# aliftffd/ViT-vs-Raw-IQ

Measured on AMD Instinct MI355X. Metric: IQ frames/sec training (fwd+loss+bwd+clip+AdamW), higher is better.
Workload: dtype bf16; 1 GPU; ViT-Tiny/16 224x224 C=1 19cls (BASELINE configs[1]); config_id=B, per_gpu_batch=256, global_batch=256, parallelism=dp1, hipgraph=True

## Files before the change

vit-vs-raw-iq_amd/csrc/attention.hip:

```cpp
#include <stdlib.h>

#include "common.h"
#include "iqvit.h"
#include "prof.h"

namespace {

constexpr int ATT_THREADS = 512;
constexpr int ATT_WAVES = ATT_THREADS / 64;
constexpr float LOG2E = 1.4426950408889634f;
constexpr float LN2 = 0.6931471805599453f;
constexpr float NEG_BIG = -1.0e30f;

__device__ __forceinline__ float fast_exp2(float x) { return __builtin_amdgcn_exp2f(x); }

template <int DH> struct AttCfg {
  static constexpr int LD = (DH == 16) ? 16 : DH + 16;
  static constexpr int KS = (DH + 31) / 32;
  static constexpr int DT = DH / 16;
  static constexpr int CPR = DH / 8;
};

typedef __attribute__((address_space(3))) s16x4 lds_s16x4;

__device__ __forceinline__ bf16x8 tr_frag(const bf16* tile, int ld, int r0, int c0, int lane) {
  const int i16 = lane & 15, g = lane >> 4;
  const bf16* a = tile + (r0 + 4 * g + (i16 >> 2)) * ld + c0 + 4 * (i16 & 3);
  s16x4 lo = __builtin_amdgcn_ds_read_tr16_b64_v4i16((lds_s16x4*)(a));
  s16x4 hi = __builtin_amdgcn_ds_read_tr16_b64_v4i16((lds_s16x4*)(a + 16 * ld));
  s16x8 v = {lo[0], lo[1], lo[2], lo[3], hi[0], hi[1], hi[2], hi[3]};
  return __builtin_bit_cast(bf16x8, v);
}

template <int DH>
__device__ __forceinline__ bf16x8 row_frag_lds(const bf16* tile, int row, int s, int lane) {
  const int d0 = s * 32 + 8 * (lane >> 4);
  bf16x8 v = {};
  if (DH >= 32 || d0 < DH) v = *reinterpret_cast<const bf16x8*>(tile + row * AttCfg<DH>::LD + d0);
  return v;
}
template <int DH>
__device__ __forceinline__ bf16x8 row_frag_gmem(const bf16* base, long ldg, int row, int nrows, int s, int lane) {
  const int d0 = s * 32 + 8 * (lane >> 4);
  bf16x8 v = {};
  if (row < nrows && (DH >= 32 || d0 < DH)) v = *reinterpret_cast<const bf16x8*>(base + (long)row * ldg + d0);
  return v;
}

template <int DH>
__device__ __forceinline__ void stage_rows(bf16* img, const bf16* base, long ldg, int r_begin, int nrows_pad, int S,
                                           int tid) {
  constexpr int CPR = AttCfg<DH>::CPR, LD = AttCfg<DH>::LD;
  for (int id = tid; id < nrows_pad * CPR; id += ATT_THREADS) {
    const int r = id / CPR, c = id % CPR;
    bf16x8 v = {};
    if (r_begin + r < S) v = *reinterpret_cast<const bf16x8*>(base + (long)(r_begin + r) * ldg + c * 8);
    *reinterpret_cast<bf16x8*>(img + r * LD + c * 8) = v;
  }
}

template <int DH, int UN>
__device__ __forceinline__ void stage_pair(bf16* imgA, const bf16* baseA, long ldgA, bf16* imgB, const bf16* baseB, long ldgB,
                                           int r_begin, int nrows_pad, int S, int tid) {
  constexpr int CPR = AttCfg<DH>::CPR, LD = AttCfg<DH>::LD;
  const int total = nrows_pad * CPR;
  for (int base = 0; base < total; base += UN * ATT_THREADS) {
    bf16x8 va[UN], vb[UN];
#pragma unroll
    for (int j = 0; j < UN; ++j) {
      const int id = min(base + j * ATT_THREADS + tid, total - 1);
      const int r = min(r_begin + id / CPR, S - 1), c = id % CPR;
      va[j] = *reinterpret_cast<const bf16x8*>(baseA + (long)r * ldgA + c * 8);
      vb[j] = *reinterpret_cast<const bf16x8*>(baseB + (long)r * ldgB + c * 8);
    }
#pragma unroll
    for (int j = 0; j < UN; ++j) {
      const int id = base + j * ATT_THREADS + tid;
      const int r = id / CPR, c = id % CPR;
      if (id < total) {
        const bool live = r_begin + r < S;
        *reinterpret_cast<bf16x8*>(imgA + r * LD + c * 8) = live ? va[j] : bf16x8{};
        *reinterpret_cast<bf16x8*>(imgB + r * LD + c * 8) = live ? vb[j] : bf16x8{};
      }
    }
  }
}

__device__ __forceinline__ bf16x8 pack_b(const f32x4& lo, const f32x4& hi) {
  bf16x8 v;
#pragma unroll
  for (int r = 0; r < 4; ++r) { v[r] = (bf16)lo[r]; v[4 + r] = (bf16)hi[r]; }
  return v;
}

__device__ __forceinline__ float group4_max(float v) {
  v = fmaxf(v, __shfl_xor(v, 16, 64));
  return fmaxf(v, __shfl_xor(v, 32, 64));
}
__device__ __forceinline__ float group4_sum(float v) {
  v += __shfl_xor(v, 16, 64);
  return v + __shfl_xor(v, 32, 64);
}

template <int DH, bool MASKED>
__global__ __launch_bounds__(ATT_THREADS) void attn_fwd_kernel(const bf16* __restrict__ qkv, bf16* __restrict__ out,
                                                               float* __restrict__ lse, const uint8_t* __restrict__ mask,
                                                               long mask_hstride, int S, int H, int kchunk,
                                                               float scale_log2, float masked_raw) {
  using C = AttCfg<DH>;
  extern __shared__ __attribute__((aligned(16))) unsigned char smem[];
  bf16* Ks = reinterpret_cast<bf16*>(smem);
  bf16* Vs = Ks + kchunk * C::LD;
  const int tid = threadIdx.x, lane = tid & 63, wave = tid >> 6, g = lane >> 4, c16 = lane & 15;
  const int b = blockIdx.x / H, h = blockIdx.x % H;
  const int D = H * DH;
  const long ldg = 3L * D;
  const bf16* qb = qkv + (long)b * S * ldg + h * DH;
  const bf16* kb_ = qb + D;
  const bf16* vb_ = qb + 2 * D;
  const uint8_t* mk = MASKED ? mask + (long)b * (mask_hstride ? (long)H * S * S : (long)S * S) + h * mask_hstride : nullptr;
  const int qtiles = (S + 31) / 32, npass = (qtiles + ATT_WAVES - 1) / ATT_WAVES, nstage = (S + kchunk - 1) / kchunk;

  if (nstage == 1) {
    stage_pair<DH, 4>(Ks, kb_, ldg, Vs, vb_, ldg, 0, min(kchunk, ((S + 31) / 32) * 32), S, tid);
    __syncthreads();
  }
  for (int pass = 0; pass < npass; ++pass) {
    const int qt = pass * ATT_WAVES + wave;
    const bool active = qt < qtiles;
    bf16x8 qf[2][C::KS];
    f32x4 o[2][C::DT];
    float m[2], lsum[2];
#pragma unroll
    for (int u = 0; u < 2; ++u) {
      m[u] = NEG_BIG; lsum[u] = 0.f;
#pragma unroll
      for (int s = 0; s < C::KS; ++s) qf[u][s] = row_frag_gmem<DH>(qb, ldg, qt * 32 + u * 16 + c16, active ? S : 0, s, lane);
#pragma unroll
      for (int dt = 0; dt < C::DT; ++dt) o[u][dt] = f32x4{0.f, 0.f, 0.f, 0.f};
    }
    for (int st = 0; st < nstage; ++st) {
      const int k0 = st * kchunk;
      const int krows = min(kchunk, ((S - k0 + 31) / 32) * 32);
      if (nstage > 1) {
        __syncthreads();
        stage_pair<DH, 2>(Ks, kb_, ldg, Vs, vb_, ldg, k0, krows, S, tid);
        __syncthreads();
      }
      if (active) {
        const bool u1 = qt * 32 + 16 < S;
        for (int kb = 0; kb < krows; kb += 32) {
          const bool k1 = k0 + kb + 16 < S;
          const bool kpad = k0 + kb + 32 > S;
          f32x4 sc[2][2];
#pragma unroll
          for (int kt = 0; kt < 2; ++kt) {
            if (kt == 1 && !k1) {
              sc[0][1] = f32x4{0.f, 0.f, 0.f, 0.f}; sc[1][1] = f32x4{0.f, 0.f, 0.f, 0.f};
              continue;
            }
            bf16x8 kf[C::KS];
#pragma unroll
            for (int s = 0; s < C::KS; ++s) kf[s] = row_frag_lds<DH>(Ks, kb + kt * 16 + c16, s, lane);
#pragma unroll
            for (int u = 0; u < 2; ++u) {
              f32x4 a = {0.f, 0.f, 0.f, 0.f};
              if (u == 0 || u1) {
#pragma unroll
                for (int s = 0; s < C::KS; ++s) a = __builtin_amdgcn_mfma_f32_16x16x32_bf16(kf[s], qf[u][s], a, 0, 0, 0);
              }
              sc[u][kt] = a;
            }
          }
          bf16x8 pb[2];
#pragma unroll
          for (int u = 0; u < 2; ++u) {
            if (u == 1 && !u1) { pb[1] = bf16x8{}; continue; }
            float mx = NEG_BIG;
#pragma unroll
            for (int kt = 0; kt < 2; ++kt) {
              if (kt == 1 && !k1) continue;
#pragma unroll
              for (int r = 0; r < 4; ++r) {
                float x = sc[u][kt][r];
                if (MASKED) {
                  const int key = k0 + kb + kt * 16 + 4 * g + r;
                  const int q = qt * 32 + u * 16 + c16;
                  if (key < S && q < S && !mk[(long)q * S + key]) x = masked_raw;
                }
                if (kpad) {
                  const int key = k0 + kb + kt * 16 + 4 * g + r;
                  x = key < S ? x : NEG_BIG;
                }
                sc[u][kt][r] = x;
                mx = fmaxf(mx, x);
              }
            }
            mx = group4_max(mx) * scale_log2;
            const float mn = fmaxf(m[u], mx);
            const float alpha = fast_exp2(m[u] - mn);
            m[u] = mn;
            float rs = 0.f;
#pragma unroll
            for (int kt = 0; kt < 2; ++kt) {
              if (kt == 1 && !k1) continue;
#pragma unroll
              for (int r = 0; r < 4; ++r) {
                const float pv = fast_exp2(fmaf(sc[u][kt][r], scale_log2, -mn));
                sc[u][kt][r] = pv;
                rs += pv;
              }
            }
            lsum[u] = lsum[u] * alpha + rs;
#pragma unroll
            for (int dt = 0; dt < C::DT; ++dt) o[u][dt] *= alpha;
            pb[u] = pack_b(sc[u][0], sc[u][1]);
          }
#pragma unroll
          for (int dt = 0; dt < C::DT; ++dt) {
            const bf16x8 vt = tr_frag(Vs, C::LD, kb, dt * 16, lane);
            o[0][dt] = __builtin_amdgcn_mfma_f32_16x16x32_bf16(vt, pb[0], o[0][dt], 0, 0, 0);
            if (u1) o[1][dt] = __builtin_amdgcn_mfma_f32_16x16x32_bf16(vt, pb[1], o[1][dt], 0, 0, 0);
          }
        }
      }
    }
    if (active) {
#pragma unroll
      for (int u = 0; u < 2; ++u) {
        const float l = group4_sum(lsum[u]);
        const float inv = 1.0f / l;
        const int q = qt * 32 + u * 16 + c16;
        if (q < S) {
#pragma unroll
          for (int dt = 0; dt < C::DT; ++dt) {
            bf16x4 w;
#pragma unroll
            for (int r = 0; r < 4; ++r) w[r] = (bf16)(o[u][dt][r] * inv);
            *reinterpret_cast<bf16x4*>(out + ((long)b * S + q) * D + h * DH + dt * 16 + 4 * g) = w;
          }
          if (g == 0) lse[((long)b * H + h) * S + q] = (m[u] + log2f(l)) * LN2;
        }
      }
    }
  }
}

template <int DH, bool MASKED>
__global__ __launch_bounds__(ATT_THREADS, 4) void attn_bwd_kernel(const bf16* __restrict__ qkv, const bf16* __restrict__ out,
                                                               const bf16* __restrict__ dout, const float* __restrict__ lse,
                                                               bf16* __restrict__ dqkv, const uint8_t* __restrict__ mask,
                                                               long mask_hstride, int S, int H, int spad, int chunk,
                                                               float scale, float masked_raw) {
  using C = AttCfg<DH>;
  extern __shared__ __attribute__((aligned(16))) unsigned char smem[];
  bf16* I0 = reinterpret_cast<bf16*>(smem);
  bf16* I1 = I0 + chunk * C::LD;
  float* lse_s = reinterpret_cast<float*>(I1 + chunk * C::LD);
  float* del_s = lse_s + spad;
  const int tid = threadIdx.x, lane = tid & 63, wave = tid >> 6, g = lane >> 4, c16 = lane & 15;
  const int b = blockIdx.x / H, h = blockIdx.x % H;
  const int D = H * DH;
  const long ldg = 3L * D;
  const bf16* qb = qkv + (long)b * S * ldg + h * DH;
  const bf16* kb_ = qb + D;
  const bf16* vb_ = qb + 2 * D;
  const bf16* ob = out + (long)b * S * D + h * DH;
  const bf16* dob = dout + (long)b * S * D + h * DH;
  bf16* dqb = dqkv + (long)b * S * ldg + h * DH;
  const uint8_t* mk = MASKED ? mask + (long)b * (mask_hstride ? (long)H * S * S : (long)S * S) + h * mask_hstride : nullptr;
  const float scale_log2 = scale * LOG2E;
  const int nblk = spad / 32;
  const int nchunk = (spad + chunk - 1) / chunk;
  const bool single = nchunk == 1;

  if (single) {
    stage_pair<DH, 4>(I0, qb, ldg, I1, dob, (long)D, 0, spad, S, tid);
    __syncthreads();
  }
  for (int q = tid; q < spad; q += ATT_THREADS) {
    float dl = 0.f, ls = 0.f;
    if (q < S) {
#pragma unroll
      for (int c = 0; c < C::CPR; ++c) {
        const bf16x8 a = single ? *reinterpret_cast<const bf16x8*>(I1 + q * C::LD + c * 8)
                                : *reinterpret_cast<const bf16x8*>(dob + (long)q * D + c * 8);
        const bf16x8 o8 = *reinterpret_cast<const bf16x8*>(ob + (long)q * D + c * 8);
#pragma unroll
        for (int e = 0; e < 8; ++e) dl += (float)a[e] * (float)o8[e];
      }
      ls = lse[((long)b * H + h) * S + q] * LOG2E;
    }
    del_s[q] = dl;
    lse_s[q] = ls;
  }
  __syncthreads();

  const int nunit = (S + 15) / 16;
  for (int ug = 0; ug * ATT_WAVES < nunit; ++ug) {
    const int unit = ug * ATT_WAVES + wave;
    const bool have = unit < nunit;
    bf16x8 kf[C::KS], vf[C::KS];
#pragma unroll
    for (int s = 0; s < C::KS; ++s) {
      kf[s] = row_frag_gmem<DH>(kb_, ldg, unit * 16 + c16, have ? S : 0, s, lane);
      vf[s] = row_frag_gmem<DH>(vb_, ldg, unit * 16 + c16, have ? S : 0, s, lane);
    }
    f32x4 dv[C::DT], dk[C::DT];
#pragma unroll
    for (int dt = 0; dt < C::DT; ++dt) { dv[dt] = f32x4{0.f, 0.f, 0.f, 0.f}; dk[dt] = f32x4{0.f, 0.f, 0.f, 0.f}; }
    const int key = unit * 16 + c16;
    const bool unit_partial = unit * 16 + 16 > S;
    for (int qc = 0; qc < nchunk; ++qc) {
      const int q0 = qc * chunk;
      const int rows = min(chunk, spad - q0);
      if (!single) {
        __syncthreads();
        stage_pair<DH, 2>(I0, qb, ldg, I1, dob, (long)D, q0, rows, S, tid);
        __syncthreads();
      }
      if (!have) continue;
      for (int ql = 0; ql < rows; ql += 32) {
        const bool u1 = q0 + ql + 16 < S;
        f32x4 p[2], ds[2];
#pragma unroll
        for (int u = 0; u < 2; ++u) {
          if (u == 1 && !u1) { p[1] = f32x4{0.f, 0.f, 0.f, 0.f}; ds[1] = f32x4{0.f, 0.f, 0.f, 0.f}; continue; }
          f32x4 sa = {0.f, 0.f, 0.f, 0.f}, dp = {0.f, 0.f, 0.f, 0.f};
#pragma unroll
          for (int s = 0; s < C::KS; ++s) {
            const bf16x8 qa = row_frag_lds<DH>(I0, ql + u * 16 + c16, s, lane);
            const bf16x8 da = row_frag_lds<DH>(I1, ql + u * 16 + c16, s, lane);
            sa = __builtin_amdgcn_mfma_f32_16x16x32_bf16(qa, kf[s], sa, 0, 0, 0);
            dp = __builtin_amdgcn_mfma_f32_16x16x32_bf16(da, vf[s], dp, 0, 0, 0);
          }
#pragma unroll
          for (int r = 0; r < 4; ++r) {
            const int q = q0 + ql + u * 16 + 4 * g + r;
            bool blocked = false;
            if (MASKED) blocked = q < S && key < S && !mk[(long)q * S + key];
            float pv = fast_exp2((blocked ? masked_raw : sa[r]) * scale_log2 - lse_s[q]);
            if (unit_partial) pv = key < S ? pv : 0.f;
            p[u][r] = pv;
            ds[u][r] = blocked ? 0.f : pv * (dp[r] - del_s[q]) * scale;
          }
        }
        const bf16x8 pB = pack_b(p[0], p[1]), dsB = pack_b(ds[0], ds[1]);
#pragma unroll
        for (int dt = 0; dt < C::DT; ++dt) {
          const bf16x8 doT = tr_frag(I1, C::LD, ql, dt * 16, lane);
          const bf16x8 qT = tr_frag(I0, C::LD, ql, dt * 16, lane);
          dv[dt] = __builtin_amdgcn_mfma_f32_16x16x32_bf16(doT, pB, dv[dt], 0, 0, 0);
          dk[dt] = __builtin_amdgcn_mfma_f32_16x16x32_bf16(qT, dsB, dk[dt], 0, 0, 0);
        }
      }
    }
    if (have && key < S) {
#pragma unroll
      for (int dt = 0; dt < C::DT; ++dt) {
        bf16x4 wk, wv;
#pragma unroll
        for (int r = 0; r < 4; ++r) { wk[r] = (bf16)dk[dt][r]; wv[r] = (bf16)dv[dt][r]; }
        *reinterpret_cast<bf16x4*>(dqb + (long)key * ldg + D + dt * 16 + 4 * g) = wk;
        *reinterpret_cast<bf16x4*>(dqb + (long)key * ldg + 2 * D + dt * 16 + 4 * g) = wv;
      }
    }
  }

  bf16x8 qf[2][C::KS], dof[2][C::KS];
  if (single) {
#pragma unroll
    for (int u = 0; u < 2; ++u)
#pragma unroll
      for (int s = 0; s < C::KS; ++s) {
        const int q = min(wave, nblk - 1) * 32 + u * 16 + c16;
        qf[u][s] = row_frag_lds<DH>(I0, q, s, lane);
        dof[u][s] = row_frag_lds<DH>(I1, q, s, lane);
      }
  }
  for (int qg = 0; qg * ATT_WAVES < nblk; ++qg) {
    const int qblk = qg * ATT_WAVES + wave;
    const bool have = qblk < nblk;
    float lq[2], dl[2];
#pragma unroll
    for (int u = 0; u < 2; ++u) {
      const int q = min(qblk, nblk - 1) * 32 + u * 16 + c16;
      if (!single || qg != 0) {
#pragma unroll
        for (int s = 0; s < C::KS; ++s) {
          qf[u][s] = row_frag_gmem<DH>(qb, ldg, q, have ? S : 0, s, lane);
          dof[u][s] = row_frag_gmem<DH>(dob, (long)D, q, have ? S : 0, s, lane);
        }
      }
      lq[u] = lse_s[q];
      dl[u] = del_s[q];
    }
    f32x4 dq[C::DT][2];
#pragma unroll
    for (int dt = 0; dt < C::DT; ++dt)
#pragma unroll
      for (int u = 0; u < 2; ++u) dq[dt][u] = f32x4{0.f, 0.f, 0.f, 0.f};
    for (int kc = 0; kc < nchunk; ++kc) {
      const int k0 = kc * chunk;
      const int rows = min(chunk, spad - k0);
      if (!single || qg == 0) {
        __syncthreads();
        stage_pair<DH, 2>(I0, kb_, ldg, I1, vb_, ldg, k0, rows, S, tid);
        __syncthreads();
      }
      if (!have) continue;
      const bool u1 = qblk * 32 + 16 < S;
      for (int kl = 0; kl < rows; kl += 32) {
        const bool kblk_partial = k0 + kl + 32 > S;
        const bool k1 = k0 + kl + 16 < S;
        f32x4 ds[2][2];
#pragma unroll
        for (int kt = 0; kt < 2; ++kt) {
          if (kt == 1 && !k1) { ds[0][1] = f32x4{0.f, 0.f, 0.f, 0.f}; ds[1][1] = f32x4{0.f, 0.f, 0.f, 0.f}; continue; }
          bf16x8 ka[C::KS], va[C::KS];
#pragma unroll
          for (int s = 0; s < C::KS; ++s) {
            ka[s] = row_frag_lds<DH>(I0, kl + kt * 16 + c16, s, lane);
            va[s] = row_frag_lds<DH>(I1, kl + kt * 16 + c16, s, lane);
          }
#pragma unroll
          for (int u = 0; u < 2; ++u) {
            if (u == 1 && !u1) { ds[1][kt] = f32x4{0.f, 0.f, 0.f, 0.f}; continue; }
            f32x4 sa = {0.f, 0.f, 0.f, 0.f}, dp = {0.f, 0.f, 0.f, 0.f};
#pragma unroll
            for (int s = 0; s < C::KS; ++s) {
              sa = __builtin_amdgcn_mfma_f32_16x16x32_bf16(ka[s], qf[u][s], sa, 0, 0, 0);
              dp = __builtin_amdgcn_mfma_f32_16x16x32_bf16(va[s], dof[u][s], dp, 0, 0, 0);
            }
#pragma unroll
            for (int r = 0; r < 4; ++r) {
              const int key = k0 + kl + kt * 16 + 4 * g + r;
              bool blocked = false;
              if (MASKED) {
                const int q = qblk * 32 + u * 16 + c16;
                blocked = q < S && key < S && !mk[(long)q * S + key];
              }
              float pv = fast_exp2((blocked ? masked_raw : sa[r]) * scale_log2 - lq[u]);
              if (kblk_partial) pv = key < S ? pv : 0.f;
              ds[u][kt][r] = blocked ? 0.f : pv * (dp[r] - dl[u]) * scale;
            }
          }
        }
        bf16x8 dsB[2];
#pragma unroll
        for (int u = 0; u < 2; ++u) dsB[u] = pack_b(ds[u][0], ds[u][1]);
#pragma unroll
        for (int dt = 0; dt < C::DT; ++dt) {
          const bf16x8 kT = tr_frag(I0, C::LD, kl, dt * 16, lane);
          dq[dt][0] = __builtin_amdgcn_mfma_f32_16x16x32_bf16(kT, dsB[0], dq[dt][0], 0, 0, 0);
          if (u1) dq[dt][1] = __builtin_amdgcn_mfma_f32_16x16x32_bf16(kT, dsB[1], dq[dt][1], 0, 0, 0);
        }
      }
    }
    if (have) {
#pragma unroll
      for (int u = 0; u < 2; ++u) {
        const int q = qblk * 32 + u * 16 + c16;
        if (q < S) {
#pragma unroll
          for (int dt = 0; dt < C::DT; ++dt) {
            bf16x4 w;
#pragma unroll
            for (int r = 0; r < 4; ++r) w[r] = (bf16)dq[dt][u][r];
            *reinterpret_cast<bf16x4*>(dqb + (long)q * ldg + dt * 16 + 4 * g) = w;
          }
        }
      }
    }
  }
}

constexpr int ONCE_MAX_SPAD = 224;
constexpr int ONCE_LD = 64;

__device__ __forceinline__ int once_off(int row, int col) { return row * ONCE_LD + (col ^ (((row >> 1) & 3) << 4)); }

__device__ __forceinline__ bf16x8 once_tr_frag(const bf16* tile, int r0, int dt, int lane) {
  const int i16 = lane & 15, g = lane >> 4;
  const bf16* a = tile + once_off(r0 + 4 * g + (i16 >> 2), dt * 16 + 4 * (i16 & 3));
  s16x4 lo = __builtin_amdgcn_ds_read_tr16_b64_v4i16((lds_s16x4*)(a));
  s16x4 hi = __builtin_amdgcn_ds_read_tr16_b64_v4i16((lds_s16x4*)(a + 16 * ONCE_LD));
  s16x8 v = {lo[0], lo[1], lo[2], lo[3], hi[0], hi[1], hi[2], hi[3]};
  return __builtin_bit_cast(bf16x8, v);
}
__device__ __forceinline__ bf16x8 once_row_frag(const bf16* tile, int row, int s, int lane) {
  return *reinterpret_cast<const bf16x8*>(tile + once_off(row, s * 32 + 8 * (lane >> 4)));
}

template <int NT, int UN, int NIMG>
__device__ __forceinline__ void once_stage(bf16* const (&img)[NIMG], const bf16* const (&base)[NIMG],
                                           const long (&ldg)[NIMG], int spad, int S, int tid) {
  const int total = spad * 8;
  for (int b0 = 0; b0 < total; b0 += UN * NT) {
    bf16x8 v[NIMG][UN];
#pragma unroll
    for (int j = 0; j < UN; ++j) {
      const int id = min(b0 + j * NT + tid, total - 1);
      const int r = min(id >> 3, S - 1), c = id & 7;
#pragma unroll
      for (int i = 0; i < NIMG; ++i) v[i][j] = *reinterpret_cast<const bf16x8*>(base[i] + (long)r * ldg[i] + c * 8);
    }
#pragma unroll
    for (int j = 0; j < UN; ++j) {
      const int id = b0 + j * NT + tid;
      const int r = id >> 3, c = id & 7;
      if (id < total) {
        const bool live = r < S;
#pragma unroll
        for (int i = 0; i < NIMG; ++i) *reinterpret_cast<bf16x8*>(img[i] + once_off(r, c * 8)) = live ? v[i][j] : bf16x8{};
      }
    }
  }
}

template <int NT>
__global__ __launch_bounds__(NT, 4) void attn_bwd_once_kernel(const bf16* __restrict__ qkv, const bf16* __restrict__ out,
                                                              const bf16* __restrict__ dout, const float* __restrict__ lse,
                                                              bf16* __restrict__ dqkv, int S, int H, int spad, float scale) {
  constexpr int DH = 64, KS = 2, DT = 4, NW = NT / 64;
  extern __shared__ __attribute__((aligned(16))) unsigned char smem[];
  bf16* I0 = reinterpret_cast<bf16*>(smem);
  bf16* I1 = I0 + spad * ONCE_LD;
  float* lse_s = reinterpret_cast<float*>(I1 + spad * ONCE_LD);
  float* del_s = lse_s + spad;
  bf16* dSi = reinterpret_cast<bf16*>(del_s + spad);
  const int tid = threadIdx.x, lane = tid & 63, wave = tid >> 6, g = lane >> 4, c16 = lane & 15;
  const int b = blockIdx.x / H, h = blockIdx.x % H;
  const int D = H * DH;
  const long ldg = 3L * D;
  const bf16* qb = qkv + (long)b * S * ldg + h * DH;
  const bf16* kb_ = qb + D;
  const bf16* vb_ = qb + 2 * D;
  const bf16* ob = out + (long)b * S * D + h * DH;
  const bf16* dob = dout + (long)b * S * D + h * DH;
  bf16* dqb = dqkv + (long)b * S * ldg + h * DH;
  const float scale_log2 = scale * LOG2E;
  const int nunit = (S + 15) / 16;
  const int ldS = nunit * 16 + 8;

  {
    bf16* const img[2] = {I0, I1};
    const bf16* const src[2] = {qb, dob};
    const long lds_[2] = {ldg, (long)D};
    once_stage<NT, 2048 / NT, 2>(img, src, lds_, spad, S, tid);
  }
  __syncthreads();
  for (int q = tid; q < spad; q += NT) {
    float dl = 0.f, ls = 0.f;
    if (q < S) {
#pragma unroll
      for (int c = 0; c < 8; ++c) {
        const bf16x8 a = *reinterpret_cast<const bf16x8*>(I1 + once_off(q, c * 8));
        const bf16x8 o8 = *reinterpret_cast<const bf16x8*>(ob + (long)q * D + c * 8);
#pragma unroll
        for (int e = 0; e < 8; ++e) dl += (float)a[e] * (float)o8[e];
      }
      ls = lse[((long)b * H + h) * S + q] * LOG2E;
    }
    del_s[q] = dl;
    lse_s[q] = ls;
  }
  __syncthreads();

  for (int unit = wave; unit < nunit; unit += NW) {
    bf16x8 kf[KS], vf[KS];
#pragma unroll
    for (int s = 0; s < KS; ++s) {
      kf[s] = row_frag_gmem<DH>(kb_, ldg, unit * 16 + c16, S, s, lane);
      vf[s] = row_frag_gmem<DH>(vb_, ldg, unit * 16 + c16, S, s, lane);
    }
    f32x4 dv[DT], dk[DT];
#pragma unroll
    for (int dt = 0; dt < DT; ++dt) { dv[dt] = f32x4{0.f, 0.f, 0.f, 0.f}; dk[dt] = f32x4{0.f, 0.f, 0.f, 0.f}; }
    const int key = unit * 16 + c16;
    const bool unit_partial = unit * 16 + 16 > S;
    for (int ql = 0; ql < spad; ql += 32) {
      const bool u1 = ql + 16 < S;
      f32x4 p[2], ds[2];
#pragma unroll
      for (int u = 0; u < 2; ++u) {
        if (u == 1 && !u1) { p[1] = f32x4{0.f, 0.f, 0.f, 0.f}; ds[1] = f32x4{0.f, 0.f, 0.f, 0.f}; continue; }
        f32x4 sa = {0.f, 0.f, 0.f, 0.f}, dp = {0.f, 0.f, 0.f, 0.f};
#pragma unroll
        for (int s = 0; s < KS; ++s) {
          const bf16x8 qa = once_row_frag(I0, ql + u * 16 + c16, s, lane);
          const bf16x8 da = once_row_frag(I1, ql + u * 16 + c16, s, lane);
          sa = __builtin_amdgcn_mfma_f32_16x16x32_bf16(qa, kf[s], sa, 0, 0, 0);
          dp = __builtin_amdgcn_mfma_f32_16x16x32_bf16(da, vf[s], dp, 0, 0, 0);
        }
        const f32x4 lq4 = *reinterpret_cast<const f32x4*>(lse_s + ql + u * 16 + 4 * g);
        const f32x4 dl4 = *reinterpret_cast<const f32x4*>(del_s + ql + u * 16 + 4 * g);
#pragma unroll
        for (int r = 0; r < 4; ++r) {
          float pv = fast_exp2(sa[r] * scale_log2 - lq4[r]);
          if (unit_partial) pv = key < S ? pv : 0.f;
          p[u][r] = pv;
          ds[u][r] = pv * (dp[r] - dl4[r]) * scale;
        }
      }
      const bf16x8 pB = pack_b(p[0], p[1]), dsB = pack_b(ds[0], ds[1]);
      bf16* w = dSi + (ql + 4 * g) * ldS + key;
#pragma unroll
      for (int r = 0; r < 4; ++r) w[r * ldS] = dsB[r];
      if (u1) {
#pragma unroll
        for (int r = 0; r < 4; ++r) w[(16 + r) * ldS] = dsB[4 + r];
      }
#pragma unroll
      for (int dt = 0; dt < DT; ++dt) {
        const bf16x8 doT = once_tr_frag(I1, ql, dt, lane);
        const bf16x8 qT = once_tr_frag(I0, ql, dt, lane);
        dv[dt] = __builtin_amdgcn_mfma_f32_16x16x32_bf16(doT, pB, dv[dt], 0, 0, 0);
        dk[dt] = __builtin_amdgcn_mfma_f32_16x16x32_bf16(qT, dsB, dk[dt], 0, 0, 0);
      }
    }
    if (key < S) {
#pragma unroll
      for (int dt = 0; dt < DT; ++dt) {
        bf16x4 wk, wv;
#pragma unroll
        for (int r = 0; r < 4; ++r) { wk[r] = (bf16)dk[dt][r]; wv[r] = (bf16)dv[dt][r]; }
        *reinterpret_cast<bf16x4*>(dqb + (long)key * ldg + D + dt * 16 + 4 * g) = wk;
        *reinterpret_cast<bf16x4*>(dqb + (long)key * ldg + 2 * D + dt * 16 + 4 * g) = wv;
      }
    }
  }

  __syncthreads();
  {
    bf16* const img[1] = {I0};
    const bf16* const src[1] = {kb_};
    const long lds_[1] = {ldg};
    once_stage<NT, 2048 / NT, 1>(img, src, lds_, spad, S, tid);
  }
  __syncthreads();
  for (int half = wave; half < nunit; half += NW) {
    const int q = half * 16 + c16;
    const bf16* drow = dSi + q * ldS + 4 * g;
    f32x4 dq[DT];
#pragma unroll
    for (int dt = 0; dt < DT; ++dt) dq[dt] = f32x4{0.f, 0.f, 0.f, 0.f};
    for (int kl = 0; kl < spad; kl += 32) {
      const bool k1 = kl + 16 < S;
      const bf16x4 lo = *reinterpret_cast<const bf16x4*>(drow + kl);
      bf16x4 hi = {};
      if (k1) hi = *reinterpret_cast<const bf16x4*>(drow + kl + 16);
      const bf16x8 dsB = {lo[0], lo[1], lo[2], lo[3], hi[0], hi[1], hi[2], hi[3]};
#pragma unroll
      for (int dt = 0; dt < DT; ++dt) {
        const bf16x8 kT = once_tr_frag(I0, kl, dt, lane);
        dq[dt] = __builtin_amdgcn_mfma_f32_16x16x32_bf16(kT, dsB, dq[dt], 0, 0, 0);
      }
    }
    if (q < S) {
#pragma unroll
      for (int dt = 0; dt < DT; ++dt) {
        bf16x4 w;
#pragma unroll
        for (int r = 0; r < 4; ++r) w[r] = (bf16)dq[dt][r];
        *reinterpret_cast<bf16x4*>(dqb + (long)q * ldg + dt * 16 + 4 * g) = w;
      }
    }
  }
}

template <int DH>
__device__ __forceinline__ bf16x8 row_frag_img(const bf16* tile, int ld, int row, int s, int lane) {
  const int d0 = s * 32 + 8 * (lane >> 4);
  bf16x8 v = {};
  if (DH >= 32 || d0 < DH) v = *reinterpret_cast<const bf16x8*>(tile + row * ld + d0);
  return v;
}

template <int UN>
__device__ __forceinline__ void stage_block(bf16* img, int ld, const bf16* src, int cols, int S, int spad, int tid, int nthr) {
  const int cpr = cols >> 3, total = spad * cpr, live = S * cpr;
  for (int base = 0; base < total; base += UN * nthr) {
    bf16x8 v[UN];
#pragma unroll
    for (int j = 0; j < UN; ++j) {
      const int id = min(base + j * nthr + tid, live - 1);
      v[j] = *reinterpret_cast<const bf16x8*>(src + (long)id * 8);
    }
#pragma unroll
    for (int j = 0; j < UN; ++j) {
      const int id = base + j * nthr + tid;
      if (id < total) {
        const int r = id / cpr, c = id - r * cpr;
        *reinterpret_cast<bf16x8*>(img + r * ld + c * 8) = id < live ? v[j] : bf16x8{};
      }
    }
  }
}

template <int DH, int G>
__global__ __launch_bounds__(ATT_THREADS) void attn_frame_fwd_kernel(const bf16* __restrict__ qkv, bf16* __restrict__ out,
                                                                     float* __restrict__ lse, int S, int H, int spad,
                                                                     float scale_log2) {
  using C = AttCfg<DH>;
  extern __shared__ __attribute__((aligned(16))) unsigned char smem[];
  bf16* img = reinterpret_cast<bf16*>(smem);
  const int tid = threadIdx.x, lane = tid & 63, wave = tid >> 6, g = lane >> 4, c16 = lane & 15;
  const int nwave = blockDim.x >> 6;
  const int b = blockIdx.x;
  const int D = H * DH, ld = 3 * D + 16;
  stage_block<8>(img, ld, qkv + (long)b * S * 3 * D, 3 * D, S, spad, tid, blockDim.x);
  __syncthreads();
  const int qtiles = (S + 31) / 32;
  for (int h = wave; h < H; h += nwave) {
    const bf16* Qs = img + h * DH;
    const bf16* Ks = Qs + D;
    const bf16* Vs = Qs + 2 * D;
    for (int qt0 = 0; qt0 < qtiles; qt0 += G) {
      bf16x8 qf[G][2][C::KS];
      f32x4 o[G][2][C::DT];
      float m[G][2], lsum[G][2];
      bool live[G][2];
#pragma unroll
      for (int t = 0; t < G; ++t)
#pragma unroll
        for (int u = 0; u < 2; ++u) {
          const int q0 = (qt0 + t) * 32 + u * 16;
          live[t][u] = q0 < S;
          m[t][u] = NEG_BIG; lsum[t][u] = 0.f;
#pragma unroll
          for (int s = 0; s < C::KS; ++s) qf[t][u][s] = row_frag_img<DH>(Qs, ld, min(q0 + c16, spad - 1), s, lane);
#pragma unroll
          for (int dt = 0; dt < C::DT; ++dt) o[t][u][dt] = f32x4{0.f, 0.f, 0.f, 0.f};
        }
      for (int kb = 0; kb < spad; kb += 32) {
        const bool k1 = kb + 16 < S;
        bf16x8 kf[2][C::KS], vt[C::DT];
#pragma unroll
        for (int kt = 0; kt < 2; ++kt)
#pragma unroll
          for (int s = 0; s < C::KS; ++s) kf[kt][s] = row_frag_img<DH>(Ks, ld, kb + kt * 16 + c16, s, lane);
#pragma unroll
        for (int dt = 0; dt < C::DT; ++dt) vt[dt] = tr_frag(Vs, ld, kb, dt * 16, lane);
#pragma unroll
        for (int t = 0; t < G; ++t)
#pragma unroll
          for (int u = 0; u < 2; ++u) {
            if (!live[t][u]) continue;
            f32x4 sc[2];
#pragma unroll
            for (int kt = 0; kt < 2; ++kt) {
              f32x4 a = {0.f, 0.f, 0.f, 0.f};
              if (kt == 0 || k1) {
#pragma unroll
                for (int s = 0; s < C::KS; ++s) a = __builtin_amdgcn_mfma_f32_16x16x32_bf16(kf[kt][s], qf[t][u][s], a, 0, 0, 0);
              }
              sc[kt] = a;
            }
            float mx = NEG_BIG;
#pragma unroll
            for (int kt = 0; kt < 2; ++kt) {
              if (kt == 1 && !k1) { sc[1] = f32x4{0.f, 0.f, 0.f, 0.f}; continue; }
#pragma unroll
              for (int r = 0; r < 4; ++r) {
                const int key = kb + kt * 16 + 4 * g + r;
                const float x = key < S ? sc[kt][r] : NEG_BIG;
                sc[kt][r] = x;
                mx = fmaxf(mx, x);
              }
            }
            mx = group4_max(mx) * scale_log2;
            const float mn = fmaxf(m[t][u], mx);
            const float alpha = fast_exp2(m[t][u] - mn);
            m[t][u] = mn;
            float rs = 0.f;
#pragma unroll
            for (int kt = 0; kt < 2; ++kt) {
              if (kt == 1 && !k1) continue;
#pragma unroll
              for (int r = 0; r < 4; ++r) {
                const float pv = fast_exp2(fmaf(sc[kt][r], scale_log2, -mn));
                sc[kt][r] = pv;
                rs += pv;
              }
            }
            lsum[t][u] = lsum[t][u] * alpha + rs;
            const bf16x8 pb = pack_b(sc[0], sc[1]);
#pragma unroll
            for (int dt = 0; dt < C::DT; ++dt) {
              o[t][u][dt] *= alpha;
              o[t][u][dt] = __builtin_amdgcn_mfma_f32_16x16x32_bf16(vt[dt], pb, o[t][u][dt], 0, 0, 0);
            }
          }
      }
#pragma unroll
      for (int t = 0; t < G; ++t)
#pragma unroll
        for (int u = 0; u < 2; ++u) {
          if (!live[t][u]) continue;
          const float l = group4_sum(lsum[t][u]);
          const float inv = 1.0f / l;
          const int q = (qt0 + t) * 32 + u * 16 + c16;
          if (q < S) {
#pragma unroll
            for (int dt = 0; dt < C::DT; ++dt) {
              bf16x4 w;
#pragma unroll
              for (int r = 0; r < 4; ++r) w[r] = (bf16)(o[t][u][dt][r] * inv);
              *reinterpret_cast<bf16x4*>(out + ((long)b * S + q) * D + h * DH + dt * 16 + 4 * g) = w;
            }
            if (g == 0) lse[((long)b * H + h) * S + q] = (m[t][u] + log2f(l)) * LN2;
          }
        }
    }
  }
}

template <int DH, int UG, int QG>
__global__ __launch_bounds__(ATT_THREADS) void attn_frame_bwd_kernel(const bf16* __restrict__ qkv, const bf16* __restrict__ out,
                                                                     const bf16* __restrict__ dout, const float* __restrict__ lse,
                                                                     bf16* __restrict__ dqkv, int S, int H, int spad, float scale) {
  using C = AttCfg<DH>;
  extern __shared__ __attribute__((aligned(16))) unsigned char smem[];
  const int tid = threadIdx.x, lane = tid & 63, wave = tid >> 6, g = lane >> 4, c16 = lane & 15;
  const int nwave = blockDim.x >> 6;
  const int b = blockIdx.x;
  const int D = H * DH, ld = 3 * D + 16, ldo = D + 16;
  bf16* img = reinterpret_cast<bf16*>(smem);
  bf16* dimg = img + spad * ld;
  float* lse_s = reinterpret_cast<float*>(dimg + spad * ldo);
  float* del_s = lse_s + H * spad;
  const long ldg = 3L * D;
  const float scale_log2 = scale * LOG2E;
  for (int id = tid; id < spad * H; id += blockDim.x) {
    const int q = id / H, h = id - q * H;
    float dl = 0.f, ls = 0.f;
    if (q < S) {
      const bf16* orow = out + ((long)b * S + q) * D + h * DH;
      const bf16* drow = dout + ((long)b * S + q) * D + h * DH;
#pragma unroll
      for (int c = 0; c < C::CPR; ++c) {
        const bf16x8 a = *reinterpret_cast<const bf16x8*>(drow + c * 8);
        const bf16x8 o8 = *reinterpret_cast<const bf16x8*>(orow + c * 8);
#pragma unroll
        for (int e = 0; e < 8; ++e) dl += (float)a[e] * (float)o8[e];
      }
      ls = lse[((long)b * H + h) * S + q] * LOG2E;
    }
    del_s[h * spad + q] = dl;
    lse_s[h * spad + q] = ls;
  }
  stage_block<8>(img, ld, qkv + (long)b * S * ldg, 3 * D, S, spad, tid, blockDim.x);
  stage_block<4>(dimg, ldo, dout + (long)b * S * D, D, S, spad, tid, blockDim.x);
  __syncthreads();
  bf16* dqb = dqkv + (long)b * S * ldg;
  const int nunit = (S + 15) / 16, nblk = spad / 32;
  for (int h = wave; h < H; h += nwave) {
    const bf16* Qs = img + h * DH;
    const bf16* Ks = Qs + D;
    const bf16* Vs = Qs + 2 * D;
    const bf16* Os = dimg + h * DH;
    const float* lq_s = lse_s + h * spad;
    const float* dl_s = del_s + h * spad;
    for (int un0 = 0; un0 < nunit; un0 += UG) {
      bf16x8 kf[UG][C::KS], vf[UG][C::KS];
      f32x4 dv[UG][C::DT], dk[UG][C::DT];
#pragma unroll
      for (int j = 0; j < UG; ++j) {
        const int row = min((un0 + j) * 16 + c16, spad - 1);
#pragma unroll
        for (int s = 0; s < C::KS; ++s) {
          kf[j][s] = row_frag_img<DH>(Ks, ld, row, s, lane);
          vf[j][s] = row_frag_img<DH>(Vs, ld, row, s, lane);
        }
#pragma unroll
        for (int dt = 0; dt < C::DT; ++dt) { dv[j][dt] = f32x4{0.f, 0.f, 0.f, 0.f}; dk[j][dt] = f32x4{0.f, 0.f, 0.f, 0.f}; }
      }
      for (int ql = 0; ql < spad; ql += 32) {
        const bool u1 = ql + 16 < S;
        bf16x8 qa[2][C::KS], da[2][C::KS], doT[C::DT], qT[C::DT];
        f32x4 lq4[2], dl4[2];
#pragma unroll
        for (int u = 0; u < 2; ++u) {
#pragma unroll
          for (int s = 0; s < C::KS; ++s) {
            qa[u][s] = row_frag_img<DH>(Qs, ld, ql + u * 16 + c16, s, lane);
            da[u][s] = row_frag_img<DH>(Os, ldo, ql + u * 16 + c16, s, lane);
          }
          lq4[u] = *reinterpret_cast<const f32x4*>(lq_s + ql + u * 16 + 4 * g);
          dl4[u] = *reinterpret_cast<const f32x4*>(dl_s + ql + u * 16 + 4 * g);
        }
#pragma unroll
        for (int dt = 0; dt < C::DT; ++dt) {
          doT[dt] = tr_frag(Os, ldo, ql, dt * 16, lane);
          qT[dt] = tr_frag(Qs, ld, ql, dt * 16, lane);
        }
#pragma unroll
        for (int j = 0; j < UG; ++j) {
          const int unit = un0 + j;
          if (unit >= nunit) continue;
          const int key = unit * 16 + c16;
          const bool unit_partial = unit * 16 + 16 > S;
          f32x4 p[2], ds[2];
#pragma unroll
          for (int u = 0; u < 2; ++u) {
            if (u == 1 && !u1) { p[1] = f32x4{0.f, 0.f, 0.f, 0.f}; ds[1] = f32x4{0.f, 0.f, 0.f, 0.f}; continue; }
            f32x4 sa = {0.f, 0.f, 0.f, 0.f}, dp = {0.f, 0.f, 0.f, 0.f};
#pragma unroll
            for (int s = 0; s < C::KS; ++s) {
              sa = __builtin_amdgcn_mfma_f32_16x16x32_bf16(qa[u][s], kf[j][s], sa, 0, 0, 0);
              dp = __builtin_amdgcn_mfma_f32_16x16x32_bf16(da[u][s], vf[j][s], dp, 0, 0, 0);
            }
#pragma unroll
            for (int r = 0; r < 4; ++r) {
              float pv = fast_exp2(sa[r] * scale_log2 - lq4[u][r]);
              if (unit_partial) pv = key < S ? pv : 0.f;
              p[u][r] = pv;
              ds[u][r] = pv * (dp[r] - dl4[u][r]) * scale;
            }
          }
          const bf16x8 pB = pack_b(p[0], p[1]), dsB = pack_b(ds[0], ds[1]);
#pragma unroll
          for (int dt = 0; dt < C::DT; ++dt) {
            dv[j][dt] = __builtin_amdgcn_mfma_f32_16x16x32_bf16(doT[dt], pB, dv[j][dt], 0, 0, 0);
            dk[j][dt] = __builtin_amdgcn_mfma_f32_16x16x32_bf16(qT[dt], dsB, dk[j][dt], 0, 0, 0);
          }
        }
      }
#pragma unroll
      for (int j = 0; j < UG; ++j) {
        const int key = (un0 + j) * 16 + c16;
        if (un0 + j < nunit && key < S) {
#pragma unroll
          for (int dt = 0; dt < C::DT; ++dt) {
            bf16x4 wk, wv;
#pragma unroll
            for (int r = 0; r < 4; ++r) { wk[r] = (bf16)dk[j][dt][r]; wv[r] = (bf16)dv[j][dt][r]; }
            *reinterpret_cast<bf16x4*>(dqb + (long)key * ldg + D + h * DH + dt * 16 + 4 * g) = wk;
            *reinterpret_cast<bf16x4*>(dqb + (long)key * ldg + 2 * D + h * DH + dt * 16 + 4 * g) = wv;
          }
        }
      }
    }
    for (int qb0 = 0; qb0 < nblk; qb0 += QG) {
      bf16x8 qf[QG][2][C::KS], dof[QG][2][C::KS];
      float lq[QG][2], dl[QG][2];
      bool live[QG][2];
      f32x4 dq[QG][C::DT][2];
#pragma unroll
      for (int t = 0; t < QG; ++t)
#pragma unroll
        for (int u = 0; u < 2; ++u) {
          const int q0 = (qb0 + t) * 32 + u * 16;
          live[t][u] = q0 < S;
          const int q = min(q0 + c16, spad - 1);
#pragma unroll
          for (int s = 0; s < C::KS; ++s) {
            qf[t][u][s] = row_frag_img<DH>(Qs, ld, q, s, lane);
            dof[t][u][s] = row_frag_img<DH>(Os, ldo, q, s, lane);
          }
          lq[t][u] = lq_s[q];
          dl[t][u] = dl_s[q];
#pragma unroll
          for (int dt = 0; dt < C::DT; ++dt) dq[t][dt][u] = f32x4{0.f, 0.f, 0.f, 0.f};
        }
      for (int kl = 0; kl < spad; kl += 32) {
        const bool kblk_partial = kl + 32 > S;
        const bool k1 = kl + 16 < S;
        bf16x8 ka[2][C::KS], va[2][C::KS], kT[C::DT];
#pragma unroll
        for (int kt = 0; kt < 2; ++kt)
#pragma unroll
          for (int s = 0; s < C::KS; ++s) {
            ka[kt][s] = row_frag_img<DH>(Ks, ld, kl + kt * 16 + c16, s, lane);
            va[kt][s] = row_frag_img<DH>(Vs, ld, kl + kt * 16 + c16, s, lane);
          }
#pragma unroll
        for (int dt = 0; dt < C::DT; ++dt) kT[dt] = tr_frag(Ks, ld, kl, dt * 16, lane);
#pragma unroll
        for (int t = 0; t < QG; ++t)
#pragma unroll
          for (int u = 0; u < 2; ++u) {
            if (!live[t][u]) continue;
            f32x4 ds[2];
#pragma unroll
            for (int kt = 0; kt < 2; ++kt) {
              if (kt == 1 && !k1) { ds[1] = f32x4{0.f, 0.f, 0.f, 0.f}; continue; }
              f32x4 sa = {0.f, 0.f, 0.f, 0.f}, dp = {0.f, 0.f, 0.f, 0.f};
#pragma unroll
              for (int s = 0; s < C::KS; ++s) {
                sa = __builtin_amdgcn_mfma_f32_16x16x32_bf16(ka[kt][s], qf[t][u][s], sa, 0, 0, 0);
                dp = __builtin_amdgcn_mfma_f32_16x16x32_bf16(va[kt][s], dof[t][u][s], dp, 0, 0, 0);
              }
#pragma unroll
              for (int r = 0; r < 4; ++r) {
                const int key = kl + kt * 16 + 4 * g + r;
                float pv = fast_exp2(sa[r] * scale_log2 - lq[t][u]);
                if (kblk_partial) pv = key < S ? pv : 0.f;
                ds[kt][r] = pv * (dp[r] - dl[t][u]) * scale;
              }
            }
            const bf16x8 dsB = pack_b(ds[0], ds[1]);
#pragma unroll
            for (int dt = 0; dt < C::DT; ++dt)
              dq[t][dt][u] = __builtin_amdgcn_mfma_f32_16x16x32_bf16(kT[dt], dsB, dq[t][dt][u], 0, 0, 0);
          }
      }
#pragma unroll
      for (int t = 0; t < QG; ++t)
#pragma unroll
        for (int u = 0; u < 2; ++u) {
          const int q = (qb0 + t) * 32 + u * 16 + c16;
          if (live[t][u] && q < S) {
#pragma unroll
            for (int dt = 0; dt < C::DT; ++dt) {
              bf16x4 w;
#pragma unroll
              for (int r = 0; r < 4; ++r) w[r] = (bf16)dq[t][dt][u][r];
              *reinterpret_cast<bf16x4*>(dqb + (long)q * ldg + h * DH + dt * 16 + 4 * g) = w;
            }
          }
        }
    }
  }
}

constexpr size_t ATT_FRAME_LDS_MAX = 112 * 1024;
inline size_t frame_fwd_lds(int S, int H, int dh) {
  const int spad = (S + 31) / 32 * 32;
  return (size_t)spad * (3 * H * dh + 16) * 2;
}
inline size_t frame_bwd_lds(int S, int H, int dh) {
  const int spad = (S + 31) / 32 * 32;
  return (size_t)spad * (3 * H * dh + 16) * 2 + (size_t)spad * (H * dh + 16) * 2 + (size_t)2 * H * spad * sizeof(float);
}
inline bool use_frame(int S, size_t lds) {
  static const int tune = [] { const char* e = getenv("IQ_TUNE_ATTN_FRAME"); return e ? atoi(e) : -1; }();
  if (lds > ATT_FRAME_LDS_MAX) return false;
  if (tune == 0) return false;
  if (tune == 1) return true;
  return S <= 128;
}

template <int DH>
int launch_frame_fwd(const void* qkv, void* out, float* lse, int B, int S, int H, hipStream_t st) {
  const int spad = (S + 31) / 32 * 32;
  const size_t lds = frame_fwd_lds(S, H, DH);
  auto k = attn_frame_fwd_kernel<DH, (DH == 64 ? 2 : 4)>;
  if (lds > 48 * 1024) (void)hipFuncSetAttribute((const void*)k, hipFuncAttributeMaxDynamicSharedMemorySize, (int)lds);
  const int threads = 64 * (H < ATT_WAVES ? H : ATT_WAVES);
  k<<<B, threads, lds, st>>>((const bf16*)qkv, (bf16*)out, lse, S, H, spad, LOG2E / sqrtf((float)DH));
  return iq_launch_status();
}
template <int DH>
int launch_frame_bwd(const void* qkv, const void* out, const void* dout, const float* lse, void* dqkv, int B, int S, int H,
                     hipStream_t st) {
  const int spad = (S + 31) / 32 * 32;
  const size_t lds = frame_bwd_lds(S, H, DH);
  auto k = attn_frame_bwd_kernel<DH, (DH == 64 ? 2 : 3), (DH == 16 ? 4 : DH == 32 ? 3 : 2)>;
  if (lds > 48 * 1024) (void)hipFuncSetAttribute((const void*)k, hipFuncAttributeMaxDynamicSharedMemorySize, (int)lds);
  const int threads = 64 * (H < ATT_WAVES ? H : ATT_WAVES);
  k<<<B, threads, lds, st>>>((const bf16*)qkv, (const bf16*)out, (const bf16*)dout, lse, (bf16*)dqkv, S, H, spad,
                             1.0f / sqrtf((float)DH));
  return iq_launch_status();
}

constexpr size_t ATT_LDS_FWD_BUDGET = 72 * 1024;
constexpr size_t ATT_LDS_BWD_BUDGET = 76 * 1024;
constexpr int ATT_MAX_S = 4096;

template <int DH> int bwd_chunk_rows(int S) {
  const int spad = (S + 31) / 32 * 32;
  const long room = (long)ATT_LDS_BWD_BUDGET - (long)2 * spad * sizeof(float);
  int chunk = (int)(room / (2 * AttCfg<DH>::LD * 2)) / 32 * 32;
  if (chunk > spad) chunk = spad;
  return chunk;
}
template <int DH> size_t bwd_lds_bytes(int S) {
  const int spad = (S + 31) / 32 * 32;
  return (size_t)2 * bwd_chunk_rows<DH>(S) * AttCfg<DH>::LD * 2 + (size_t)2 * spad * sizeof(float);
}

template <int DH, bool MASKED>
int launch_fwd(const void* qkv, void* out, float* lse, const uint8_t* mask, long mask_hstride, int B, int S, int H,
               hipStream_t st) {
  const int spad = (S + 31) / 32 * 32;
  int kchunk = (int)(ATT_LDS_FWD_BUDGET / (2 * AttCfg<DH>::LD * 2)) / 32 * 32;
  if (kchunk > spad) kchunk = spad;
  const size_t lds = (size_t)2 * kchunk * AttCfg<DH>::LD * 2;
  const float scale_log2 = LOG2E / sqrtf((float)DH);
  if (lds > 48 * 1024)
    (void)hipFuncSetAttribute((const void*)attn_fwd_kernel<DH, MASKED>, hipFuncAttributeMaxDynamicSharedMemorySize, (int)lds);
  attn_fwd_kernel<DH, MASKED><<<B * H, ATT_THREADS, lds, st>>>((const bf16*)qkv, (bf16*)out, lse, mask, mask_hstride, S, H,
                                                               kchunk, scale_log2, -10000.0f * sqrtf((float)DH));
  return iq_launch_status();
}

template <int DH, bool MASKED>
int launch_bwd(const void* qkv, const void* out, const void* dout, const float* lse, void* dqkv, const uint8_t* mask,
               long mask_hstride, int B, int S, int H, hipStream_t st) {
  const int spad = (S + 31) / 32 * 32;
  const int chunk = bwd_chunk_rows<DH>(S);
  if (S > ATT_MAX_S || chunk < 32) return IQ_ERR_UNSUPPORTED;
  const size_t lds = bwd_lds_bytes<DH>(S);
  if (lds > 48 * 1024)
    (void)hipFuncSetAttribute((const void*)attn_bwd_kernel<DH, MASKED>, hipFuncAttributeMaxDynamicSharedMemorySize, (int)lds);
  attn_bwd_kernel<DH, MASKED><<<B * H, ATT_THREADS, lds, st>>>((const bf16*)qkv, (const bf16*)out, (const bf16*)dout, lse,
                                                               (bf16*)dqkv, mask, mask_hstride, S, H, spad, chunk,
                                                               1.0f / sqrtf((float)DH), -10000.0f * sqrtf((float)DH));
  return iq_launch_status();
}

inline int once_threads(int S, int dh, bool masked) {
  static const int tune = [] { const char* e = getenv("IQ_TUNE_ATTN_BWD_ONCE"); return e ? atoi(e) : -1; }();
  if (masked || dh != 64 || (S + 31) / 32 * 32 > ONCE_MAX_SPAD || tune == 0) return 0;
  return tune == 512 ? 512 : 1024;
}
template <int NT>
int launch_bwd_once(const void* qkv, const void* out, const void* dout, const float* lse, void* dqkv, int B, int S, int H,
                    hipStream_t st) {
  const int spad = (S + 31) / 32 * 32, nunit = (S + 15) / 16;
  const size_t lds = (size_t)2 * spad * ONCE_LD * 2 + (size_t)2 * spad * sizeof(float) + (size_t)spad * (nunit * 16 + 8) * 2;
  auto k = attn_bwd_once_kernel<NT>;
  if (lds > 48 * 1024) (void)hipFuncSetAttribute((const void*)k, hipFuncAttributeMaxDynamicSharedMemorySize, (int)lds);
  k<<<B * H, NT, lds, st>>>((const bf16*)qkv, (const bf16*)out, (const bf16*)dout, lse, (bf16*)dqkv, S, H, spad,
                            1.0f / sqrtf(64.0f));
  return iq_launch_status();
}

template <bool MASKED>
int dispatch_fwd(const void* qkv, void* out, float* lse, const uint8_t* mask, long hs, int B, int S, int H, int dh,
                 hipStream_t st) {
  switch (dh) {
    case 16: return launch_fwd<16, MASKED>(qkv, out, lse, mask, hs, B, S, H, st);
    case 32: return launch_fwd<32, MASKED>(qkv, out, lse, mask, hs, B, S, H, st);
    case 64: return launch_fwd<64, MASKED>(qkv, out, lse, mask, hs, B, S, H, st);
    default: return IQ_ERR_UNSUPPORTED;
  }
}
template <bool MASKED>
int dispatch_bwd(const void* qkv, const void* out, const void* dout, const float* lse, void* dqkv, const uint8_t* mask,
                 long hs, int B, int S, int H, int dh, hipStream_t st) {
  switch (dh) {
    case 16: return launch_bwd<16, MASKED>(qkv, out, dout, lse, dqkv, mask, hs, B, S, H, st);
    case 32: return launch_bwd<32, MASKED>(qkv, out, dout, lse, dqkv, mask, hs, B, S, H, st);
    case 64: return launch_bwd<64, MASKED>(qkv, out, dout, lse, dqkv, mask, hs, B, S, H, st);
    default: return IQ_ERR_UNSUPPORTED;
  }
}

}

extern "C" int iq_attn_supported(int S, int dh) {
  if (S <= 0 || S > ATT_MAX_S) return 0;
  return (dh == 16 || dh == 32 || dh == 64) ? 1 : 0;
}

extern "C" int iq_attn_fwd_masked(const void* qkv, void* out, float* lse, const uint8_t* mask, long mask_hstride, int B,
                                  int S, int H, int dh, iq_stream_t stream) {
  if (B <= 0) return IQ_OK;
  if (!qkv || !out || !lse || S <= 0 || H <= 0) return IQ_ERR_ARG;
  if (mask_hstride != 0 && mask_hstride != (long)S * S) return IQ_ERR_ARG;
  hipStream_t st = (hipStream_t)stream;
  IQ_PROF(IQ_FAM_ATTN_FWD, st);
  const bool frame = !mask && (dh == 16 || dh == 32 || dh == 64) && use_frame(S, frame_fwd_lds(S, H, dh));
  {
    const double rows = (double)B * S, Dm = (double)H * dh;
    if (frame) IQ_PROF_K(2.0 * rows * 4.0 * Dm + 4.0 * B * H * S, 4.0 * B * H * (double)S * S * dh, "attn_frame_fwd_kernel<%d>", dh);
    else IQ_PROF_K(2.0 * rows * 4.0 * Dm + 4.0 * B * H * S, 4.0 * B * H * (double)S * S * dh, "attn_fwd_kernel<%d, %s>", dh, mask ? "true" : "false");
  }
  if (frame) {
    switch (dh) {
      case 16: return launch_frame_fwd<16>(qkv, out, lse, B, S, H, st);
      case 32: return launch_frame_fwd<32>(qkv, out, lse, B, S, H, st);
      default: return launch_frame_fwd<64>(qkv, out, lse, B, S, H, st);
    }
  }
  return mask ? dispatch_fwd<true>(qkv, out, lse, mask, mask_hstride, B, S, H, dh, st)
              : dispatch_fwd<false>(qkv, out, lse, nullptr, 0, B, S, H, dh, st);
}
extern "C" int iq_attn_fwd(const void* qkv, void* out, float* lse, int B, int S, int H, int dh, iq_stream_t stream) {
  return iq_attn_fwd_masked(qkv, out, lse, nullptr, 0, B, S, H, dh, stream);
}

extern "C" int iq_attn_bwd_masked(const void* qkv, const void* out, const void* dout, const float* lse, void* dqkv,
                                  const uint8_t* mask, long mask_hstride, int B, int S, int H, int dh,
                                  iq_stream_t stream) {
  if (B <= 0) return IQ_OK;
  if (!qkv || !out || !dout || !lse || !dqkv || S <= 0 || H <= 0) return IQ_ERR_ARG;
  if (mask_hstride != 0 && mask_hstride != (long)S * S) return IQ_ERR_ARG;
  hipStream_t st = (hipStream_t)stream;
  IQ_PROF(IQ_FAM_ATTN_BWD, st);
  const bool frame = !mask && (dh == 16 || dh == 32 || dh == 64) && use_frame(S, frame_bwd_lds(S, H, dh));
  const int once = frame ? 0 : once_threads(S, dh, mask != nullptr);
  {
    const double rows = (double)B * S, Dm = (double)H * dh;
    if (frame) IQ_PROF_K(2.0 * rows * 8.0 * Dm + 4.0 * B * H * S, 14.0 * B * H * (double)S * S * dh, "attn_frame_bwd_kernel<%d>", dh);
    else if (once) IQ_PROF_K(2.0 * rows * 8.0 * Dm + 4.0 * B * H * S, 10.0 * B * H * (double)S * S * dh, "attn_bwd_once_kernel<%d>", once);
    else IQ_PROF_K(2.0 * rows * 8.0 * Dm + 4.0 * B * H * S, 14.0 * B * H * (double)S * S * dh, "attn_bwd_kernel<%d, %s>", dh, mask ? "true" : "false");
  }
  if (frame) {
    switch (dh) {
      case 16: return launch_frame_bwd<16>(qkv, out, dout, lse, dqkv, B, S, H, st);
      case 32: return launch_frame_bwd<32>(qkv, out, dout, lse, dqkv, B, S, H, st);
      default: return launch_frame_bwd<64>(qkv, out, dout, lse, dqkv, B, S, H, st);
    }
  }
  if (once == 512) return launch_bwd_once<512>(qkv, out, dout, lse, dqkv, B, S, H, st);
  if (once) return launch_bwd_once<1024>(qkv, out, dout, lse, dqkv, B, S, H, st);
  return mask ? dispatch_bwd<true>(qkv, out, dout, lse, dqkv, mask, mask_hstride, B, S, H, dh, st)
              : dispatch_bwd<false>(qkv, out, dout, lse, dqkv, nullptr, 0, B, S, H, dh, st);
}
extern "C" int iq_attn_bwd(const void* qkv, const void* out, const void* dout, const float* lse, void* dqkv, int B,
                           int S, int H, int dh, iq_stream_t stream) {
  return iq_attn_bwd_masked(qkv, out, dout, lse, dqkv, nullptr, 0, B, S, H, dh, stream);
}
```

Baseline: 52430 frames/s.

## Prefetch K/V fragments, O tile and LSE early in attention backward kernel

```diff
diff --git a/vit-vs-raw-iq_amd/csrc/attention.hip b/vit-vs-raw-iq_amd/csrc/attention.hip
--- a/vit-vs-raw-iq_amd/csrc/attention.hip
+++ b/vit-vs-raw-iq_amd/csrc/attention.hip
@@ -495,26 +495,42 @@
 template <int NT, int UN, int NIMG>
 __device__ __forceinline__ void once_stage(bf16* const (&img)[NIMG], const bf16* const (&base)[NIMG],
                                            const long (&ldg)[NIMG], int spad, int S, int tid) {
+  static_assert(UN * NT >= ONCE_MAX_SPAD * 8, "one trip covers an image");
   const int total = spad * 8;
-  for (int b0 = 0; b0 < total; b0 += UN * NT) {
-    bf16x8 v[NIMG][UN];
-#pragma unroll
-    for (int j = 0; j < UN; ++j) {
-      const int id = min(b0 + j * NT + tid, total - 1);
-      const int r = min(id >> 3, S - 1), c = id & 7;
-#pragma unroll
-      for (int i = 0; i < NIMG; ++i) v[i][j] = *reinterpret_cast<const bf16x8*>(base[i] + (long)r * ldg[i] + c * 8);
-    }
-#pragma unroll
-    for (int j = 0; j < UN; ++j) {
-      const int id = b0 + j * NT + tid;
-      const int r = id >> 3, c = id & 7;
-      if (id < total) {
-        const bool live = r < S;
-#pragma unroll
-        for (int i = 0; i < NIMG; ++i) *reinterpret_cast<bf16x8*>(img[i] + once_off(r, c * 8)) = live ? v[i][j] : bf16x8{};
-      }
-    }
+  bf16x8 v[NIMG][UN];
+#pragma unroll
+  for (int j = 0; j < UN; ++j) {
+    const int id = min(j * NT + tid, total - 1);
+    const int r = min(id >> 3, S - 1), c = id & 7;
+#pragma unroll
+    for (int i = 0; i < NIMG; ++i) v[i][j] = *reinterpret_cast<const bf16x8*>(base[i] + (long)r * ldg[i] + c * 8);
+  }
+#pragma unroll
+  for (int j = 0; j < UN; ++j) {
+    const int id = j * NT + tid;
+    const int r = id >> 3, c = id & 7;
+    if (id < total) {
+      const bool live = r < S;
+#pragma unroll
+      for (int i = 0; i < NIMG; ++i) *reinterpret_cast<bf16x8*>(img[i] + once_off(r, c * 8)) = live ? v[i][j] : bf16x8{};
+    }
+  }
+}
+template <int NT, int UN>
+__device__ __forceinline__ void once_request(bf16x8 (&v)[UN], const bf16* base, long ldg, int spad, int S, int tid) {
+#pragma unroll
+  for (int j = 0; j < UN; ++j) {
+    const int id = min(j * NT + tid, spad * 8 - 1);
+    v[j] = *reinterpret_cast<const bf16x8*>(base + (long)min(id >> 3, S - 1) * ldg + (id & 7) * 8);
+  }
+}
+template <int NT, int UN>
+__device__ __forceinline__ void once_write(bf16* img, const bf16x8 (&v)[UN], int spad, int S, int tid) {
+#pragma unroll
+  for (int j = 0; j < UN; ++j) {
+    const int id = j * NT + tid;
+    const int r = id >> 3, c = id & 7;
+    if (id < spad * 8) *reinterpret_cast<bf16x8*>(img + once_off(r, c * 8)) = r < S ? v[j] : bf16x8{};
   }
 }
 
@@ -522,7 +538,7 @@
 __global__ __launch_bounds__(NT, 4) void attn_bwd_once_kernel(const bf16* __restrict__ qkv, const bf16* __restrict__ out,
                                                               const bf16* __restrict__ dout, const float* __restrict__ lse,
                                                               bf16* __restrict__ dqkv, int S, int H, int spad, float scale) {
-  constexpr int DH = 64, KS = 2, DT = 4, NW = NT / 64;
+  constexpr int DH = 64, KS = 2, DT = 4, NW = NT / 64, UN = 2048 / NT;
   extern __shared__ __attribute__((aligned(16))) unsigned char smem[];
   bf16* I0 = reinterpret_cast<bf16*>(smem);
   bf16* I1 = I0 + spad * ONCE_LD;
@@ -543,41 +559,57 @@
   const int nunit = (S + 15) / 16;
   const int ldS = nunit * 16 + 8;
 
+  bf16x8 kf[KS], vf[KS];
+  if (wave < nunit) {
+    const long row = min(wave * 16 + c16, S - 1);
+#pragma unroll
+    for (int s = 0; s < KS; ++s) {
+      kf[s] = *reinterpret_cast<const bf16x8*>(kb_ + row * ldg + s * 32 + 8 * g);
+      vf[s] = *reinterpret_cast<const bf16x8*>(vb_ + row * ldg + s * 32 + 8 * g);
+    }
+  }
+  const int per = (spad + NW - 1) / NW;
+  const int qd = lane < per ? wave * per + lane : spad;
+  const float ls_pre = lse[((long)b * H + h) * S + min(qd, S - 1)];
   {
-    bf16* const img[2] = {I0, I1};
-    const bf16* const src[2] = {qb, dob};
-    const long lds_[2] = {ldg, (long)D};
-    once_stage<NT, 2048 / NT, 2>(img, src, lds_, spad, S, tid);
+    bf16* const img[3] = {I0, I1, dSi};
+    const bf16* const src[3] = {qb, dob, ob};
+    const long lds_[3] = {ldg, (long)D, (long)D};
+    once_stage<NT, UN, 3>(img, src, lds_, spad, S, tid);
   }
   __syncthreads();
-  for (int q = tid; q < spad; q += NT) {
+  if (qd < spad) {
     float dl = 0.f, ls = 0.f;
-    if (q < S) {
+    if (qd < S) {
 #pragma unroll
       for (int c = 0; c < 8; ++c) {
-        const bf16x8 a = *reinterpret_cast<const bf16x8*>(I1 + once_off(q, c * 8));
-        const bf16x8 o8 = *reinterpret_cast<const bf16x8*>(ob + (long)q * D + c * 8);
+        const bf16x8 a = *reinterpret_cast<const bf16x8*>(I1 + once_off(qd, c * 8));
+        const bf16x8 o8 = *reinterpret_cast<const bf16x8*>(dSi + once_off(qd, c * 8));
 #pragma unroll
         for (int e = 0; e < 8; ++e) dl += (float)a[e] * (float)o8[e];
       }
-      ls = lse[((long)b * H + h) * S + q] * LOG2E;
-    }
-    del_s[q] = dl;
-    lse_s[q] = ls;
+      ls = ls_pre * LOG2E;
+    }
+    del_s[qd] = dl;
+    lse_s[qd] = ls;
   }
   __syncthreads();
 
   for (int unit = wave; unit < nunit; unit += NW) {
-    bf16x8 kf[KS], vf[KS];
-#pragma unroll
-    for (int s = 0; s < KS; ++s) {
-      kf[s] = row_frag_gmem<DH>(kb_, ldg, unit * 16 + c16, S, s, lane);
-      vf[s] = row_frag_gmem<DH>(vb_, ldg, unit * 16 + c16, S, s, lane);
-    }
+    const int key = unit * 16 + c16;
+    if (unit != wave) {
+      const long row = min(key, S - 1);
+#pragma unroll
+      for (int s = 0; s < KS; ++s) {
+        kf[s] = *reinterpret_cast<const bf16x8*>(kb_ + row * ldg + s * 32 + 8 * g);
+        vf[s] = *reinterpret_cast<const bf16x8*>(vb_ + row * ldg + s * 32 + 8 * g);
+      }
+    }
+#pragma unroll
+    for (int s = 0; s < KS; ++s) { kf[s] = key < S ? kf[s] : bf16x8{}; vf[s] = key < S ? vf[s] : bf16x8{}; }
     f32x4 dv[DT], dk[DT];
 #pragma unroll
     for (int dt = 0; dt < DT; ++dt) { dv[dt] = f32x4{0.f, 0.f, 0.f, 0.f}; dk[dt] = f32x4{0.f, 0.f, 0.f, 0.f}; }
-    const int key = unit * 16 + c16;
     const bool unit_partial = unit * 16 + 16 > S;
     for (int ql = 0; ql < spad; ql += 32) {
       const bool u1 = ql + 16 < S;
@@ -631,13 +663,10 @@
     }
   }
 
+  bf16x8 kpre[UN];
+  once_request<NT, UN>(kpre, kb_, ldg, spad, S, tid);
   __syncthreads();
-  {
-    bf16* const img[1] = {I0};
-    const bf16* const src[1] = {kb_};
-    const long lds_[1] = {ldg};
-    once_stage<NT, 2048 / NT, 1>(img, src, lds_, spad, S, tid);
-  }
+  once_write<NT, UN>(I0, kpre, spad, S, tid);
   __syncthreads();
   for (int half = wave; half < nunit; half += NW) {
     const int q = half * 16 + c16;
@@ -1120,7 +1149,8 @@
 int launch_bwd_once(const void* qkv, const void* out, const void* dout, const float* lse, void* dqkv, int B, int S, int H,
                     hipStream_t st) {
   const int spad = (S + 31) / 32 * 32, nunit = (S + 15) / 16;
-  const size_t lds = (size_t)2 * spad * ONCE_LD * 2 + (size_t)2 * spad * sizeof(float) + (size_t)spad * (nunit * 16 + 8) * 2;
+  const size_t dsi = max((size_t)nunit * 16 * (nunit * 16 + 8) * 2, (size_t)spad * ONCE_LD * 2);
+  const size_t lds = (size_t)2 * spad * ONCE_LD * 2 + (size_t)2 * spad * sizeof(float) + dsi;
   auto k = attn_bwd_once_kernel<NT>;
   if (lds > 48 * 1024) (void)hipFuncSetAttribute((const void*)k, hipFuncAttributeMaxDynamicSharedMemorySize, (int)lds);
   k<<<B * H, NT, lds, st>>>((const bf16*)qkv, (const bf16*)out, (const bf16*)dout, lse, (bf16*)dqkv, S, H, spad,
```

After: 51810 frames/s. -1.2%, worse.
